# ExaScience/elprep

Measured on AMD Instinct MI355X. Metric: Mreads/s through sort+markdup+BQSR, 150bp PE, higher is better.
Workload: dtype u8/int32/int64 (integer path; float64 finalize on host)

## Files before the change

### elprep_amd/csrc/bqsr.hip

```cpp
#include <utility>

#include "bqsr_common.hpp"

namespace elp {

__global__ __launch_bounds__(256) void k_pack_reference(const uint8_t *__restrict__ ascii, int64_t len, uint8_t *__restrict__ packed, int64_t packed_bytes) {
  const int64_t i = (int64_t)blockIdx.x * blockDim.x + threadIdx.x;
  if (i >= packed_bytes) return;
  uint32_t out = 0;
  for (int h = 0; h < 2; h++) {
    const int64_t j = 2 * i + h;
    uint32_t code = 8;
    if (j < len) {
      switch (ascii[j]) {
        case 'a': case 'A': case '*': code = 0; break;
        case 'c': case 'C': code = 1; break;
        case 'g': case 'G': code = 2; break;
        case 't': case 'T': code = 3; break;
        default: code = 8;
      }
    }
    out |= code << (4 * h);
  }
  packed[i] = (uint8_t)out;
// ... 102 lines not shown
  for (int q = 6; q < ELP_NQUAL; q++)
    if ((q < 64 ? (c->qual_present[0] >> q) : (c->qual_present[1] >> (q - 64))) & 1ull) quals.push_back(q);
  if (quals.empty()) quals.push_back(6);
  return quals;
}

static int rec_buffers(elp_ctx *c, const GatherScratch &S, uint32_t *block, int mode, uint32_t ncs, RecOut *ro) {
  const uint32_t nseg = mode == 2 ? std::max<uint32_t>((uint32_t)C3_NSEG, ncs) : (uint32_t)C3_NSEG;
  BqRec *recs = nullptr;
  if (mode) ELP_TRY(scratch(c, 4, S.rec_slots(mode), &recs));
  *ro = RecOut{recs, block + S.rec_cnt, block + S.seg_base, S.other_at(mode), nseg, mode == 2 ? ncs : 0u};
  if (mode) ELP_TRY(c3_segments_launch(c, S, block, nseg, ro->ncs));
  return 0;
}

static int count_one_length(elp_ctx *c, const GatherShape &g, const GatherScratch &S, const PrologueBufs &b, const RecOut &ro, const std::vector<int> &quals,
                            unsigned long long *cycle_tbl, unsigned long long *ctx_tbl) {
  const bool split = ro.ncs != 0;
  int rsw3 = 0, rlog3 = 0;
  size_t dyn3 = 0;
  (void)count3_plan(split ? 1 : g.n_cov, (int)quals.size(), g.lmax, g.lds_count3, &rsw3, &rlog3, &dyn3, g.count3_rlog);
  QMap qm;
  memset(qm.slot, 254, sizeof qm.slot);
  for (size_t s = 0; s < quals.size(); s++) qm.slot[quals[s]] = (uint8_t)s;
  const uint4 *other = reinterpret_cast<const uint4 *>(ro.recs) + 2 * (size_t)ro.other_at;
  const uint32_t *n_other = ro.cnt + (size_t)ro.nseg * C3_CSTRIDE;
  uint32_t *cw = b.block + S.cw, *ooff = cw + CO_MAXCOV;
  ELP_HIP(c, hipMemsetAsync(cw, 0, (3 * CO_MAXCOV + 1) * sizeof(uint32_t), c->stream));
  if (split) {
    uint4 *sorted = const_cast<uint4 *>(other) + 2 * (size_t)c->n;
    ELP_TRY(c3_other_sort_launch(c, other, n_other, cw, sorted));
    other = sorted;
  }
  Count3Args A3{ro.cnt, (uint32_t)C3_CSTRIDE, ro.seg_base, reinterpret_cast<const uint4 *>(ro.recs), ro.nseg, 0, (int)ro.ncs, c->uniform_len, c->qual.p,
                c->seq4.p + elp_ctx::SEQ_FRONT, reinterpret_cast<const uint8_t *>(b.skipbits), reinterpret_cast<const uint4 *>(b.desc), c->cigar.p, b.cs_pool,
                c->d_ref_seq.p, c->d_ref_seq_len.p, g.n_cov, (int)quals.size(), g.lmax, g.max_cycle, rsw3, rlog3, cycle_tbl, ctx_tbl, c->err_flag.p};
  ELP_TRY(count3_launch(c, A3, qm, dyn3));
  A3.other = 1;
  A3.srecs = other;
  A3.seg_base = ooff;
  A3.cnt_stride = 1;
  if (split) { A3.seg_cnt = cw; A3.nseg = ro.ncs; }
  else { A3.seg_cnt = n_other; A3.nseg = 1; }
  return count3_launch(c, A3, qm, dyn3);
}

static int count_general(elp_ctx *c, const GatherShape &g, const CountPlan &p, const PrologueBufs &b, const std::vector<int> &quals,
                         unsigned long long *cycle_tbl, unsigned long long *ctx_tbl) {
  for (int cov0 = 0; cov0 < g.n_cov; cov0 += p.ncp)
    for (size_t q0 = 0; q0 < quals.size(); q0 += (size_t)p.qcap) {
      const int nqs = (int)std::min<size_t>((size_t)p.qcap, quals.size() - q0), ncov_pass = std::min(p.ncp, g.n_cov - cov0);
      QMap qm;
      memset(qm.slot, 254, sizeof qm.slot);
      for (int q : quals) qm.slot[q] = 255;
      for (int s = 0; s < nqs; s++) qm.slot[quals[q0 + s]] = (uint8_t)s;
      CountArgs A{c->n, c->qual_bytes, c->qual_off.p, c->seq_off.p, c->qual.p, c->seq4.p, b.desc, c->cigar.p, b.cs_pool,
                  reinterpret_cast<const uint8_t *>(b.skipbits), c->d_ref_seq.p, c->d_ref_seq_len.p, c->n_ref, ncov_pass, nqs, g.lmax, p.rs, g.max_cycle,
                  cycle_tbl, ctx_tbl, c->err_flag.p, c->tile_first.p, cov0};
      ELP_TRY(count_general_launch(c, A, qm, p, p.dyn(ncov_pass, nqs)));
    }
  return 0;
}

static int tables_to_host(elp_ctx *c, size_t nq, size_t nc, size_t nx, int64_t *qual_tbl, int64_t *cycle_tbl, int64_t *ctx_tbl) {
  const size_t bytes = (nq + nc + nx) * 8;
  if (bytes > c->h_pinned_cap) {
    if (c->h_pinned) (void)hipHostFree(c->h_pinned);
// ... 233 lines not shown
```

### elprep_amd/csrc/bqsr_common.hpp

```cpp
#pragma once
#include "apply_plan.hpp"
#include "bqsr_dev.hpp"
#include "bqsr_plan.hpp"
#include "flat.hpp"

namespace elp {

constexpr int MAX_DESC_READ = 65535;


constexpr int32_t BQ_NOREF = INT32_MIN;
enum : uint8_t { BQ_ELIGIBLE = 1, BQ_REVERSED = 2, BQ_LAST = 4, BQ_CIG_SCRATCH = 8, BQ_COMPLEX = 16 };
struct __attribute__((aligned(16))) BqDesc {
  int32_t D0, D1, D2;
  int32_t refid;
  uint16_t b1, b2;
  uint16_t a;
  uint16_t len;
  uint16_t left;
  uint16_t right;
  uint8_t cov;
  uint8_t fl;
  uint16_t pad;
};
// ... 192 lines not shown
  if (!general && any_ref) {
    if (P.np > 1 && !(nr & 2u)) { const int64_t d = P.v1 - vf; general |= d < -16 || d > 14; d1 = (int)d; }
    if (P.np > 2 && !(nr & 4u)) { const int64_t d = P.v2 - vf; general |= d < -16 || d > 14; d2 = (int)d; }
    if (P.np > 3 && !(nr & 8u)) { const int64_t d = P.v3 - vf; general |= d < -16 || d > 14; d3 = (int)d; }
    general |= E0 < 16 || E0 + lorig > rlen + 32;
  }
  general |= !any_ref;
  if (general) {
    fl |= RC_GENERAL;
    r.bpk = 0x3FFFFFFFu; r.dpk = 0;
  } else {
    fl |= (nr & 0xFu) << 24;
    if (P.np > 1 || (nr & 1u)) fl |= RC_MULTI;
    r.bpk = (uint32_t)(P.np > 1 ? P.s1 : 1023) | ((uint32_t)(P.np > 2 ? P.s2 : 1023) << 10) | ((uint32_t)(P.np > 3 ? P.s3 : 1023) << 20);
    r.dpk = ((uint32_t)d1 & 0xFFu) | (((uint32_t)d2 & 0xFFu) << 8) | (((uint32_t)d3 & 0xFFu) << 16);
    fl |= (E0 & 1) ? RC_PAR : 0u;
  }
  const uint64_t pq = reinterpret_cast<uint64_t>(general ? rp : rp + (E0 >> 1) - 8);
  r.ref_lo = (uint32_t)pq;
  r.ref_hi = (uint32_t)(pq >> 32);
  r.fl = fl;
  return r;
}

struct Count3Args {
  const uint32_t *seg_cnt;
  uint32_t cnt_stride;
  const uint32_t *seg_base;
  const uint4 *srecs;
  uint32_t nseg;
  int other;
  int ncs;
  uint32_t len;
  const uint8_t *qual, *seq4;
  const uint8_t *skipbits;
  const uint4 *desc;
  const uint32_t *cigar, *cig_scratch;
  uint8_t *const *ref_seq;
  const int64_t *ref_seq_len;
  int n_cov, n_q, lmax, max_cycle;
  int rsw, rlog;
  unsigned long long *cycle_tbl, *ctx_tbl;
  uint32_t *err;
};
int count3_launch(elp_ctx *c, const Count3Args &A, const QMap &qm, size_t dyn);

struct CountArgs {
  uint64_t n, qual_bytes;
  const uint64_t *qual_off, *seq_off;
  const uint8_t *qual, *seq4;
  const BqDesc *desc;
  const uint32_t *cigar, *cig_scratch;
  const uint8_t *skipbits;
  uint8_t *const *ref_seq;
  const int64_t *ref_seq_len;
  int n_ref, n_cov, n_q, lmax, rs, max_cycle;
  unsigned long long *cycle_tbl, *ctx_tbl;
  uint32_t *err;
  const uint32_t *tile_first;
  int cov0;
};

int count_general_launch(elp_ctx *c, const CountArgs &A, const QMap &qm, const CountPlan &p, size_t dyn);
int qual_from_cycle_launch(elp_ctx *c, int ncyc_g, const unsigned long long *cycle_tbl, unsigned long long *qual_tbl);
int c3_segments_launch(elp_ctx *c, const GatherScratch &S, uint32_t *block, uint32_t nseg, uint32_t ncs);
int c3_other_sort_launch(elp_ctx *c, const uint4 *other, const uint32_t *n_other, uint32_t *cw, uint4 *sorted);
// ... 30 lines not shown
```

### elprep_amd/csrc/bqsr_plan.hpp

```cpp
#pragma once
#include <algorithm>
#include <cstddef>
#include <cstdint>

namespace elp {

constexpr size_t LDS_CU = 160 * 1024;

constexpr int CT_CYC = 32, CT_XROWS = 3, CT_PAD = 64;
constexpr int C3_XROWS = 3, C3_PAD = 64;
constexpr int C3_NSEG = 64;
constexpr int C3_MAXSEG = 256;
constexpr int C3_CSTRIDE = 64;
constexpr int PF_TILES = 16;
constexpr int CO_MAXCOV = 256;

inline int count3_plan(int n_cov, int n_q, int lmax, size_t static_lds, int *rsw_out, int *rlog_out, size_t *dyn_out, int force_rlog = -1) {
  const int ncw = ((17 * 2 * lmax) >> 4) + 2;
  const size_t rows = (size_t)n_cov * (size_t)(n_q + C3_XROWS);
  for (int rlog = 5; rlog >= 1; rlog--) {
    if (force_rlog >= 0 && force_rlog != rlog) continue;
    const int rsw = ((16 << rlog) + 16 + ncw + 31) & ~31;
    const size_t dyn = (rows * (size_t)rsw + C3_PAD) * 4;
    if (dyn + static_lds <= LDS_CU && rows * (size_t)rsw * 4 < (1u << 22)) {
      *rsw_out = rsw; *rlog_out = rlog; *dyn_out = dyn;
      return 0;
    }
  }
  return 1;
}

struct GatherShape {
  int n_cov, lmax, max_cycle;
  uint32_t uniform_len;
  int count_kernel, count3_rlog;
  size_t lds_count3, lds_count, lds_count1024;
};

inline int c3_mode(const GatherShape &g, int nq) {
  if (g.count_kernel == 1 || g.uniform_len == 0 || g.lmax > g.max_cycle || g.lmax > 1022) return 0;
  int rsw = 0, rlog = 0;
  size_t dyn = 0;
  const bool all_fits = count3_plan(g.n_cov, nq, g.lmax, g.lds_count3, &rsw, &rlog, &dyn, g.count3_rlog) == 0;
  if (all_fits && (rlog >= 3 || g.n_cov == 1) && g.count_kernel != 3) return 1;
  if (g.n_cov > 1 && g.count_kernel != 2 && count3_plan(1, nq, g.lmax, g.lds_count3, &rsw, &rlog, &dyn, g.count3_rlog) == 0) return 2;
  return all_fits ? 1 : 0;
}

struct CountPlan {
  bool fits;
  int wg_per_cu;
  bool big, mg;
  int rs;
  int ncp, qcap;
  long passes;
  size_t dyn(int ncov_pass, int nqs) const { return ((size_t)ncov_pass * (size_t)(nqs + CT_XROWS) * (size_t)rs + CT_PAD) * 4; }
};
inline int count_row_words(int lmax, bool mg) {
  const int cyc = (17 * 2 * lmax) >> 4;
  return (CT_CYC + (mg ? cyc >> 1 : cyc) + 1 + 1) & ~1;
}
inline CountPlan count_general_plan(const GatherShape &g, int nq) {
// ... 57 lines not shown
```

### elprep_amd/csrc/common.hpp

```cpp
#pragma once

#include <hip/hip_runtime.h>

#include <sched.h>

#include <cstdarg>
#include <cstdint>
#include <cstdio>
#include <cstring>
#include <map>
#include <mutex>
#include <string>
#include <vector>

#include "../../include/elprep_hip.h"
#include "../../include/elprep_hip_debug.h"
#include "apply_plan.hpp"
#include "derived.hpp"

namespace elp {

constexpr int WAVE = 64;

enum : uint16_t {
// ... 175 lines not shown
  uint64_t *presort_ks = nullptr;
  int presort_idx_bits = 0;

  elp::DVec<uint16_t> snap_flag;
  elp::DVec<uint8_t> snap_qual;
  uint64_t snap_n = 0, snap_qual_bytes = 0;

  struct Tuning {
    int count_kernel = 0;
    int apply_kernel = 0;
    int count3_rlog = -1;
    int qual_hint = 0;
    int qual_hint_drop = -1;
    int pair_table_slots = 1 << 20;
    long long bgzf_piece = 1ll << 30;
    int bgzf_weak_guess = 0;
    int score_kernel = 0;
    int mate_path = 0;
    int radix_tile = 0;
    int sort_pairs = 0;
    int tie_rounds = 0;
    int exchange_piece = 0;
    int emit_pass = 0;
    int sam_pass = 0;
    long long bgzf_inflate_piece = 2ll << 30;
    int bgzf_copy_chunk = 0;
    int bgzf_tok_lds = 0;
    int bgzf_first_chunk_div = 4;
    int bgzf_fixed = 0;
    int bgzf_tok_fail_above = 0;
    int bgzf_stored = 0;
    int apply_wgs = 0;
    int count3_grid = 0;
    int presort_tile = 0;
    int side_priority = 0;
  } tune;

  elp::DVec<uint8_t> scratch[8];

  bool profiling = false;
  const char *prof_prefix = nullptr;
  std::vector<std::string> prof_names;
  std::map<std::string, int> prof_index;
  std::vector<uint64_t> prof_launches;
  std::vector<double> prof_ms;
  std::vector<elp::ProfPending> prof_pending;
};

namespace elp {

class LaneViews {
  struct Item { void *vec; void (*take_back)(void *); };
  std::vector<Item> items;

 public:
  template <class... Col>
  LaneViews(elp_ctx *shadow, elp_ctx *ctx, Col... cols) { (view(shadow->*cols, ctx->*cols), ...); }
  LaneViews(const LaneViews &) = delete;
  LaneViews &operator=(const LaneViews &) = delete;
  ~LaneViews() {
    for (const Item &it : items) it.take_back(it.vec);
  }
  template <class T>
  void view(DVec<T> &to, const DVec<T> &from, bool with_cap = false) {
    to.p = from.p;
    to.cap = with_cap ? from.cap : 0;
// ... 212 lines not shown
```

### elprep_amd/csrc/count3.hip

```cpp
#include <algorithm>

#include "bqsr_common.hpp"
#include "gload.hpp"

namespace elp {

constexpr uint32_t N1 = 0x11111111u, C3 = 0x33333333u;
constexpr int C3_NT = 1024;

template <int BYTE>
__device__ __forceinline__ uint32_t byte_shl2(uint32_t w, uint32_t two) {
  uint32_t r;
  if (BYTE == 0) asm("v_lshlrev_b32_sdwa %0, %1, %2 dst_sel:DWORD dst_unused:UNUSED_PAD src0_sel:DWORD src1_sel:BYTE_0" : "=v"(r) : "v"(two), "v"(w));
  else if (BYTE == 1) asm("v_lshlrev_b32_sdwa %0, %1, %2 dst_sel:DWORD dst_unused:UNUSED_PAD src0_sel:DWORD src1_sel:BYTE_1" : "=v"(r) : "v"(two), "v"(w));
  else if (BYTE == 2) asm("v_lshlrev_b32_sdwa %0, %1, %2 dst_sel:DWORD dst_unused:UNUSED_PAD src0_sel:DWORD src1_sel:BYTE_2" : "=v"(r) : "v"(two), "v"(w));
  else asm("v_lshlrev_b32_sdwa %0, %1, %2 dst_sel:DWORD dst_unused:UNUSED_PAD src0_sel:DWORD src1_sel:BYTE_3" : "=v"(r) : "v"(two), "v"(w));
  return r;
}
__device__ __forceinline__ uint32_t lds_read_u32(uint32_t at) { return *reinterpret_cast<const lds_u32_t *>((uintptr_t)at); }

struct BlkRec { uint32_t win, ctxw, t0, fl, bpk, dpk; };
struct BlkData {
  u32x4 q;
  uint32_t skipw;
  u32x4 s;
  u32x4 w03;
  u32x2 w45;
};

__device__ __noinline__ uint64_t c3_ref_general(const uint4 *__restrict__ desc, const uint32_t *__restrict__ cigar, const uint32_t *__restrict__ cig_scratch,
                                               uint8_t *const *__restrict__ ref_seq, const int64_t *__restrict__ ref_seq_len, uint32_t r, uint64_t S, int blo, int bhi,
                                               int cbase) {
  const uint4 dx = desc[2 * (size_t)r], dy = desc[2 * (size_t)r + 1];
  const uint32_t dfl = (dy.w >> 8) & 0xFFu;
  const int32_t refid = (int32_t)dx.w;
  const uint8_t *__restrict__ rp = ref_seq[refid];
  const int64_t rlen = ref_seq_len[refid];
  const int32_t D0 = (int32_t)dx.x, D1 = (int32_t)dx.y, D2 = (int32_t)dx.z;
  const int b1 = (int)(dy.x & 0xFFFFu), b2 = (int)(dy.x >> 16);
  uint64_t R = 0;
  if (!(dfl & BQ_COMPLEX)) {
    const int B1 = b1 - cbase, B2 = b2 - cbase;
    {
      const int hi = bhi < B1 ? bhi : B1;
      if (blo < hi) R |= (D0 == BQ_NOREF ? S : ref_nibbles(rp, rlen, (int64_t)D0 + cbase)) & nib_fill(nib_range(blo, hi));
    }
    if (B1 < bhi) {
      const int lo = blo > B1 ? blo : B1, hi = bhi < B2 ? bhi : B2;
      if (lo < hi) R |= (D1 == BQ_NOREF ? S : ref_nibbles(rp, rlen, (int64_t)D1 + cbase)) & nib_fill(nib_range(lo, hi));
      if (B2 < bhi) {
        const int lo2 = blo > B2 ? blo : B2;
        if (lo2 < bhi) R |= (D2 == BQ_NOREF ? S : ref_nibbles(rp, rlen, (int64_t)D2 + cbase)) & nib_fill(nib_range(lo2, bhi));
      }
    }
  } else {
    const uint32_t *cg = ((dfl & BQ_CIG_SCRATCH) ? cig_scratch : cigar) + (uint32_t)D0;
    R = ref_nibbles_complex(cg, b1, (int64_t)D2, cbase, blo, bhi, rp, rlen, S);
  }
  return R;
}


template <int RLOG, bool OTHER>
struct Count3 {
  const uint8_t *__restrict__ qual;
  const uint8_t *__restrict__ seq_m1;
  const uint8_t *__restrict__ skipbits;
  const uint4 *__restrict__ desc;
  const uint32_t *__restrict__ cigar;
  const uint32_t *__restrict__ cig_scratch;
  uint8_t *const *__restrict__ ref_seq;
  const int64_t *__restrict__ ref_seq_len;
  unsigned long long *cycle_tbl, *ctx_tbl;
  uint32_t k0, nb;
  int n_cov, n_q, lmax, max_cycle, rsw;
  uint32_t qrow_at, spread_at;
  const uint8_t *slot_q;
  uint32_t *tbl;
  uint32_t rpc_bytes;
  int cov_fixed;
  int t_origin;
  uint32_t rep4, two;
  uint32_t err;

  __device__ __forceinline__ bool load_data(const u32x4 &ra, const u32x4 &rb, bool on, uint32_t len, uint32_t sbytes, BlkData &d, BlkRec &f, uint32_t &qlow,
                                            uint32_t &idx) const {
    const uint32_t a = ra.z & 0xFFFFu, e = ra.z >> 16;
    f.win = ra.z; f.ctxw = ra.w; f.t0 = rb.x; f.fl = rb.y; f.bpk = rb.z; f.dpk = rb.w;
    idx = rec_idx(ra.y, rb.y, rb.w);
    const uint64_t bit = (uint64_t)idx * len + k0;
    qlow = (uint32_t)bit & 7u;
    if (!on || k0 + nb <= a || k0 >= e) return false;
    gload_x4(d.q, (uint64_t)qual + bit);
    d.skipw = 0u;
    if (OTHER && (rb.y & RC_SKIPCOL)) gload_x1(d.skipw, (uint64_t)skipbits + (bit >> 3));
    gload_x4(d.s, (uint64_t)seq_m1 + (uint64_t)idx * sbytes + (k0 >> 1));
    const uint64_t rp = ((uint64_t)ra.x | ((uint64_t)(ra.y & 0xFFFFu) << 32)) + ((rb.y & RC_GENERAL) ? 0u : (k0 >> 1));
    gload_x4(d.w03, rp);
    gload_x2(d.w45, rp + 16);
    return true;
  }

  __device__ __forceinline__ static uint64_t win_extract(const BlkData &d, int n0) {
    uint32_t x0 = d.w03.x, x1 = d.w03.y, x2 = d.w03.z, x3 = d.w03.w, x4 = d.w45.x, x5 = d.w45.y;
    asm("" : "+v"(x0), "+v"(x1), "+v"(x2), "+v"(x3), "+v"(x4), "+v"(x5));
    const bool s16 = n0 & 16, s8 = n0 & 8;
    const uint32_t y0 = s16 ? x2 : x0, y1 = s16 ? x3 : x1, y2 = s16 ? x4 : x2, y3 = s16 ? x5 : x3;
    const uint32_t z0 = s8 ? y1 : y0, z1 = s8 ? y2 : y1, z2 = s8 ? y3 : y2;
    const uint32_t sh = 4u * (uint32_t)(n0 & 7);
    return (uint64_t)__builtin_amdgcn_alignbit(z1, z0, sh) | ((uint64_t)__builtin_amdgcn_alignbit(z2, z1, sh) << 32);
  }
  __device__ __forceinline__ static uint64_t ref_pieces(const BlkData &d, uint32_t fl, uint32_t bpk, uint32_t dpk, uint64_t S, int blo, int bhi, int cbase) {
    const int par = (fl & RC_PAR) ? 1 : 0;
    const uint32_t nr = fl >> 24;
    const int f = !(nr & 1u) ? 0 : (!(nr & 2u) ? 1 : (!(nr & 4u) ? 2 : 3));
    uint64_t R = 0;
#pragma unroll
    for (int j = 0; j < 4; j++) {
      const int bj = j == 0 ? 0 : (int)((bpk >> (10 * (j - 1))) & 1023u), bn = j == 3 ? 1023 : (int)((bpk >> (10 * j)) & 1023u);
      if (j > 0 && bj == 1023) break;
      int lo = bj - cbase, hi = bn == 1023 ? bhi : bn - cbase;
      lo = lo > blo ? lo : blo;
      hi = hi < bhi ? hi : bhi;
      if (lo < hi) {
        const int dj = j == 0 ? 0 : (int)(int8_t)((dpk >> (8 * (j - 1))) & 0xFFu);
        const uint64_t piece = ((nr >> j) & 1u) ? S : win_extract(d, 16 + par + (j == f ? 0 : dj));
        R |= piece & nib_fill(nib_range(lo, hi));
      }
    }
    return R;
  }
  template <int I>
  __device__ __forceinline__ uint32_t row_of(uint32_t qw) const { return lds_read_u32(qrow_at + byte_shl2<(I & 3)>(qw, two)); }
  template <int I>
  __device__ __forceinline__ void base(uint32_t ro, uint32_t Fh, uint32_t FVh, uint32_t CXh, uint32_t t, uint32_t lrepC) {
    constexpr int sh = 4 * (I & 7);
    lds_add_u32(lshl_add_u32<2>(t >> 4, ro), bfe_u32<sh, 1>(Fh));
    lds_add_u32(ro + lshl_add_u32<RLOG + 2>(bfe_u32<sh, 4>(CXh), lrepC), bfe_u32<sh, 1>(FVh));
  }
  __device__ __forceinline__ void mismatches(uint32_t Eh, uint32_t FVh, uint32_t CXh, uint32_t qa, uint32_t qb, uint32_t tb, int st, uint32_t rowb) {
    constexpr uint32_t cxm = (uint32_t)(16 << RLOG) * 4u;
    while (Eh) {
      const uint32_t b4 = (uint32_t)__builtin_ctz(Eh);
      const uint32_t b = b4 >> 2;
      Eh &= Eh - 1u;
      const uint32_t q = (((b & 4u) ? qb : qa) >> (8u * (b & 3u))) & 0xFFu;
      if (q < 6u) continue;
      const uint32_t ro = lds_read_u32(qrow_at + 4u * q);
      const uint32_t t = tb + (uint32_t)(st * (int)b);
      lds_add_u32(ro + ((t >> 4) << 2), 0x10000u);
      if ((FVh >> b4) & 1u) lds_add_u32(ro + rowb + cxm + (((CXh >> b4) & 15u) << 2), 1u);
    }
  }

  __device__ __forceinline__ void process(const BlkRec &f, uint32_t r, const BlkData &d, uint32_t qlow) {
    const int a = (int)(f.win & 0xFFFFu), e = (int)(f.win >> 16);
    int blo = a - (int)k0, bhi = e - (int)k0;
    blo = blo > 0 ? blo : 0;
    bhi = bhi < (int)nb ? bhi : (int)nb;
    const uint32_t fl = f.fl;
    const bool rev = fl & RC_REV;
    const uint32_t ns = rev ? 12u : 4u;
    const uint32_t S_lo = __builtin_amdgcn_alignbit(d.s.y, d.s.x, 8), S_hi = __builtin_amdgcn_alignbit(d.s.z, d.s.y, 8);
    const uint32_t N_lo = __builtin_amdgcn_alignbit(d.s.y, d.s.x, ns), N_hi = __builtin_amdgcn_alignbit(d.s.z, d.s.y, ns);
    const uint32_t oS_lo = (S_lo >> 3) & N1, oS_hi = (S_hi >> 3) & N1;
    const uint32_t oN_lo = (N_lo >> 3) & N1, oN_hi = (N_hi >> 3) & N1;
    uint32_t R_lo = 0, R_hi = 0, k_lo = 0, k_hi = 0;
    const bool one_run = !OTHER || !(fl & (RC_MULTI | RC_GENERAL));
    const bool skipcol = OTHER && (fl & RC_SKIPCOL);
    if (one_run) {
      const uint32_t sh = (fl & RC_PAR) ? 4u : 0u;
      R_lo = __builtin_amdgcn_alignbit(d.w03.w, d.w03.z, sh);
      R_hi = __builtin_amdgcn_alignbit(d.w45.x, d.w03.w, sh);
      if (!skipcol) {
        k_lo = (R_lo >> 2) & N1;
        k_hi = (R_hi >> 2) & N1;
      }
    }
    if (skipcol) {
      const uint32_t sk = d.skipw >> qlow;
      k_lo |= lds_read_u32(spread_at + ((sk & 0xFFu) << 2));
      k_hi |= lds_read_u32(spread_at + ((sk >> 6) & 0x3FCu));
    }
    const uint64_t inw = nib_range(blo, bhi);
    const uint32_t F_lo = (uint32_t)inw & ~(oS_lo | k_lo), F_hi = (uint32_t)(inw >> 32) & ~(oS_hi | k_hi);
    if ((F_lo | F_hi) == 0u) return;
    if (!one_run) {
      const uint64_t S = (uint64_t)S_lo | ((uint64_t)S_hi << 32);
      const uint64_t R = (fl & RC_GENERAL) ? c3_ref_general(desc, cigar, cig_scratch, ref_seq, ref_seq_len, r, S, blo, bhi, (int)k0 - a) : ref_pieces(d, fl, f.bpk, f.dpk, S, blo, bhi, (int)k0 - a);
      R_lo = (uint32_t)R;
      R_hi = (uint32_t)(R >> 32);
    }
    const uint32_t x_lo = S_lo ^ R_lo, x_hi = S_hi ^ R_hi;
    const uint32_t E_lo = (x_lo | (x_lo >> 1) | (x_lo >> 3)) & F_lo & N1, E_hi = (x_hi | (x_hi >> 1) | (x_hi >> 3)) & F_hi & N1;
    const uint64_t cw = nib_range_clamped((int)(f.ctxw & 0xFFFFu) - (int)k0, (int)(f.ctxw >> 16) - (int)k0);
    const uint32_t FV_lo = F_lo & (uint32_t)cw & ~oN_lo, FV_hi = F_hi & (uint32_t)(cw >> 32) & ~oN_hi;
    const uint32_t rm = rev ? 0xFFFFFFFFu : 0u;
    const uint32_t CX_lo = ((N_lo & C3) | ((S_lo & C3) << 2)) ^ rm, CX_hi = ((N_hi & C3) | ((S_hi & C3) << 2)) ^ rm;
    const int st = (fl & RC_NEG) ? -17 : 17;
    const uint32_t rowb = cov_fixed >= 0 ? 0u : __umul24(fl & 0xFFu, rpc_bytes);
    const uint32_t tb = (uint32_t)((int)f.t0 + t_origin + st * (int)k0) + 4u * rowb;
    const uint32_t lrepC = rowb + rep4;
    const uint32_t ust = (uint32_t)st;
#define ELP_B3(I, RO, FH, FVH, CXH) base<I>(RO, FH, FVH, CXH, tb + (uint32_t)(I) * ust, lrepC)
    {
      const uint32_t r0 = row_of<0>(d.q.x), r1 = row_of<1>(d.q.x), r2 = row_of<2>(d.q.x), r3 = row_of<3>(d.q.x);
      const uint32_t r4 = row_of<4>(d.q.y), r5 = row_of<5>(d.q.y), r6 = row_of<6>(d.q.y), r7 = row_of<7>(d.q.y);
      ELP_B3(0, r0, F_lo, FV_lo, CX_lo); ELP_B3(1, r1, F_lo, FV_lo, CX_lo); ELP_B3(2, r2, F_lo, FV_lo, CX_lo); ELP_B3(3, r3, F_lo, FV_lo, CX_lo);
      ELP_B3(4, r4, F_lo, FV_lo, CX_lo); ELP_B3(5, r5, F_lo, FV_lo, CX_lo); ELP_B3(6, r6, F_lo, FV_lo, CX_lo); ELP_B3(7, r7, F_lo, FV_lo, CX_lo);
      __builtin_amdgcn_sched_barrier(0);
    }
    {
      const uint32_t r0 = row_of<8>(d.q.z), r1 = row_of<9>(d.q.z), r2 = row_of<10>(d.q.z), r3 = row_of<11>(d.q.z);
      const uint32_t r4 = row_of<12>(d.q.w), r5 = row_of<13>(d.q.w), r6 = row_of<14>(d.q.w), r7 = row_of<15>(d.q.w);
      ELP_B3(8, r0, F_hi, FV_hi, CX_hi); ELP_B3(9, r1, F_hi, FV_hi, CX_hi); ELP_B3(10, r2, F_hi, FV_hi, CX_hi); ELP_B3(11, r3, F_hi, FV_hi, CX_hi);
      ELP_B3(12, r4, F_hi, FV_hi, CX_hi); ELP_B3(13, r5, F_hi, FV_hi, CX_hi); ELP_B3(14, r6, F_hi, FV_hi, CX_hi); ELP_B3(15, r7, F_hi, FV_hi, CX_hi);
      __builtin_amdgcn_sched_barrier(0);
    }
#undef ELP_B3
    {
// ... 88 lines not shown
  asm volatile("" : "+v"(B.two));
  B.err = 0;
  B.cov_fixed = A.ncs ? 0 : -1;

  const uint32_t len = A.len, bpr = (len + 15u) >> 4, sbytes = (len + 1u) >> 1, RPI = C3_NT / bpr;
  const uint32_t slot = threadIdx.x / bpr, jb = threadIdx.x - slot * bpr;
  const bool lane_on = slot < RPI;
  B.k0 = 16u * jb;
  B.nb = len - B.k0 < 16u ? len - B.k0 : 16u;
  __shared__ uint32_t s_cnt[C3_MAXSEG], s_pre[C3_MAXSEG + 1], s_wsum[4];
  static_assert(sizeof(qrow) + sizeof(spread8) + sizeof(slot_q) + sizeof(s_cnt) + sizeof(s_pre) + sizeof(s_wsum) == COUNT3_LDS_ARRAYS,
                "COUNT3_LDS_ARRAYS lists the kernel's __shared__ arrays: add a new one there too");
  {
    const uint32_t my_cnt = threadIdx.x < A.nseg ? A.seg_cnt[(size_t)threadIdx.x * A.cnt_stride] : 0u;
    const uint32_t my_trips = (my_cnt + RPI - 1u) / RPI;
    uint32_t incl = my_trips;
    for (int d = 1; d < 64; d <<= 1) {
      const uint32_t v = __shfl_up(incl, d, 64);
      if ((int)(threadIdx.x & 63u) >= d) incl += v;
    }
    if (threadIdx.x < (uint32_t)C3_MAXSEG && (threadIdx.x & 63u) == 63u) s_wsum[threadIdx.x >> 6] = incl;
    __syncthreads();
    if (threadIdx.x < (uint32_t)C3_MAXSEG) {
      uint32_t off = 0;
      for (uint32_t w = 0; w < (threadIdx.x >> 6); w++) off += s_wsum[w];
      s_cnt[threadIdx.x] = my_cnt;
      s_pre[threadIdx.x] = off + incl - my_trips;
      if (threadIdx.x == (uint32_t)C3_MAXSEG - 1u) s_pre[C3_MAXSEG] = off + incl;
    }
    __syncthreads();
  }
  const uint64_t trips_all = to_sgpr(s_pre[C3_MAXSEG]);
  const uint32_t my_lo = to_sgpr((uint32_t)(trips_all * blockIdx.x / gridDim.x)), my_hi = to_sgpr((uint32_t)(trips_all * (blockIdx.x + 1ull) / gridDim.x));
  const uint32_t flush_every = 30000u / (RPI + 1u) + 1u;
  uint64_t n = 0;
  const uint8_t *seg_recs = nullptr;
  auto first_read = [&](uint64_t it) __attribute__((always_inline)) -> uint64_t { return it * RPI; };
  const uint32_t roff = slot * 32u;
  auto rec_load = [&](uint64_t it, u32x4 &za, u32x4 &zb) __attribute__((always_inline)) {
    const uint64_t r0 = first_read(it);
    if (lane_on && r0 + slot < n) {
      const uint8_t *rt = seg_recs + r0 * 32u;
      gload_x4(za, rt, roff);
      gload_x4(zb, rt, roff + 16u);
    }
  };
  auto data_load = [&](uint64_t it, const u32x4 &za, const u32x4 &zb, BlkData &d, BlkRec &f, uint32_t &qlow, uint32_t &idx) __attribute__((always_inline)) -> bool {
    const uint64_t r0 = first_read(it);
    const bool on = lane_on && r0 + slot < n;
    return B.load_data(za, zb, on, len, sbytes, d, f, qlow, idx);
  };
  auto landed = [&](BlkData &d, const u32x4 &za, const u32x4 &zb, u32x4 &ra, u32x4 &rb) __attribute__((always_inline)) {
    gwait();
    asm volatile("" : "+v"(d.q), "+v"(d.skipw), "+v"(d.s), "+v"(d.w03), "+v"(d.w45));
    ra = amov(za);
    rb = amov(zb);
  };
  BlkData dX, dY;
  dX.q = (u32x4){0, 0, 0, 0}; dX.s = dX.q; dX.w03 = dX.q; dX.w45 = (u32x2){0, 0}; dX.skipw = 0;
  dY = dX;
  BlkRec fX, fY;
  u32x4 za = (u32x4){0, 0, 0, 0}, zb = za, na = za, nb4 = za;
  uint32_t qlX = 0, qlY = 0, iX = 0, iY = 0;
  bool onX, onY = false;
  uint32_t since = 0;
  uint32_t seg = 0;
  for (uint32_t a = 0, b = A.nseg; b - a > 1u;) {
    const uint32_t md = (a + b) >> 1;
    if (s_pre[md] <= my_lo) { a = md; seg = md; } else b = md;
  }
#pragma unroll 1
  for (; seg < A.nseg; seg++) {
    const uint32_t p0 = to_sgpr(s_pre[seg]);
    if (p0 >= my_hi) break;
    const uint32_t tr = to_sgpr(s_pre[seg + 1]) - p0, cnt_s = to_sgpr(s_cnt[seg]);
    const uint32_t t0 = my_lo > p0 ? my_lo - p0 : 0u, t1 = my_hi - p0 < tr ? my_hi - p0 : tr;
    if (t0 >= t1) continue;
    const uint64_t r_first = (uint64_t)t0 * RPI, r_end = (uint64_t)t1 * RPI < (uint64_t)cnt_s ? (uint64_t)t1 * RPI : (uint64_t)cnt_s;
    n = to_sgpr(r_end - r_first);
    seg_recs = reinterpret_cast<const uint8_t *>(to_sgpr(reinterpret_cast<uint64_t>(A.srecs) + ((uint64_t)A.seg_base[seg] + r_first) * 32u));
    const uint64_t n_trips = t1 - t0;
    B.cov_fixed = A.ncs ? (int)(seg & ((uint32_t)A.ncs - 1u)) : -1;
    rec_load(0, za, zb);
    landed(dX, za, zb, na, nb4);
    onX = data_load(0, na, nb4, dX, fX, qlX, iX);
    rec_load(1, za, zb);
    landed(dX, za, zb, na, nb4);
#pragma unroll 1
    for (uint64_t it = 0; it < n_trips; it += 2) {
      {
        onY = data_load(it + 1, na, nb4, dY, fY, qlY, iY);
        rec_load(it + 2, za, zb);
// ... 43 lines not shown
```

### elprep_amd/csrc/ctx.hip

```cpp
#include "common.hpp"

namespace elp {

namespace {
constexpr size_t GUARD = 4096;
constexpr uint8_t GUARD_BYTE = 0xC3;
std::mutex guard_mu;
std::map<void *, size_t> guard_of;
int guard_check_one(void *p, size_t payload) {
  uint8_t host[GUARD];
  if (hipDeviceSynchronize() != hipSuccess || hipMemcpy(host, static_cast<uint8_t *>(p) + payload, GUARD, hipMemcpyDeviceToHost) != hipSuccess) return 0;
  for (size_t k = 0; k < GUARD; k++)
    if (host[k] != GUARD_BYTE) {
      fprintf(stderr, "[elp] ELP_DEBUG_GUARD: byte %zu behind the end of a %zu-byte device buffer was overwritten (0x%02x)\n", k, payload, host[k]);
      return 1;
    }
  return 0;
}
}
size_t debug_guard_bytes() {
  static const size_t v = [] { const char *e = getenv("ELP_DEBUG_GUARD"); return (e && *e && *e != '0') ? GUARD : (size_t)0; }();
  return v;
}
void debug_guard_arm(void *p, size_t payload) {
// ... 568 lines not shown
  if (k == "count_kernel") c->tune.count_kernel = v;
  else if (k == "apply_kernel") c->tune.apply_kernel = v;
  else if (k == "bgzf_piece") { if (value < 1) return set_error(c, ELP_ERR_ARG, "elp_set_tuning: bgzf_piece must be positive"); c->tune.bgzf_piece = value; }
  else if (k == "bgzf_weak_guess") c->tune.bgzf_weak_guess = v;
  else if (k == "score_kernel") { c->tune.score_kernel = v; c->derived.score_tuning_changed(); }
  else if (k == "count3_rlog") c->tune.count3_rlog = v;
  else if (k == "qual_hint") { c->tune.qual_hint = v; c->derived.hint_tuning_changed(); }
  else if (k == "qual_hint_drop") { c->tune.qual_hint_drop = v; c->derived.hint_tuning_changed(); }
  else if (k == "pair_table_slots") {
    if (v == 0) { c->tune.pair_table_slots = 1 << 20; return 0; }
    if (v < 2 || v > (1 << 20) || (v & (v - 1))) return set_error(c, ELP_ERR_ARG, "elp_set_tuning: pair_table_slots must be a power of two >= 2");
    c->tune.pair_table_slots = v;
  } else if (k == "mate_path") {
    if (value != 0 && value != 2) return set_error(c, ELP_ERR_ARG, "elp_set_tuning: mate_path is 0 (the library decides) or 2 (every candidate through the table)");
    c->tune.mate_path = v;
  } else if (k == "tie_rounds") c->tune.tie_rounds = v;
  else if (k == "radix_tile") c->tune.radix_tile = v;
  else if (k == "sort_pairs") c->tune.sort_pairs = v;
  else if (k == "exchange_piece") c->tune.exchange_piece = v;
  else if (k == "emit_pass") c->tune.emit_pass = v;
  else if (k == "sam_pass") c->tune.sam_pass = v;
  else if (k == "bgzf_stored") c->tune.bgzf_stored = v;
  else if (k == "bgzf_tok_fail_above") c->tune.bgzf_tok_fail_above = v;
  else if (k == "bgzf_fixed") c->tune.bgzf_fixed = v;
  else if (k == "bgzf_first_chunk_div") c->tune.bgzf_first_chunk_div = v;
  else if (k == "bgzf_tok_lds") c->tune.bgzf_tok_lds = v;
  else if (k == "bgzf_copy_chunk") c->tune.bgzf_copy_chunk = v;
  else if (k == "bgzf_inflate_piece") { if (value < 1) return set_error(c, ELP_ERR_ARG, "elp_set_tuning: bgzf_inflate_piece must be positive"); c->tune.bgzf_inflate_piece = value; }
  else if (k == "md_fused" || k == "bgzf_inflate") {
    if (value != 0) return set_error(c, ELP_ERR_ARG, "elp_set_tuning: key '%s' is retired (only 0 is accepted)", key);
  } else if (k == "apply_wgs") c->tune.apply_wgs = v;
  else if (k == "presort_tile") c->tune.presort_tile = v;
  else if (k == "count3_grid") { if (value < 0) return set_error(c, ELP_ERR_ARG, "elp_set_tuning: count3_grid must not be negative"); c->tune.count3_grid = v; }
  else if (k == "side_priority") c->tune.side_priority = v;
  else return set_error(c, ELP_ERR_ARG, "elp_set_tuning: unknown key '%s'", key);
  return 0;
}

int elp_profile_enable(elp_ctx *c, int on) {
  if (!c) return ELP_ERR_ARG;
  if (!on) { ELP_TRY(prof_flush(c)); prof_merge_side(c); }
  c->profiling = on != 0;
  for (int lane = 0; lane < 2; lane++)
    if (c->side[lane]) c->side[lane]->profiling = c->profiling;
  return 0;
}
int elp_profile_reset(elp_ctx *c) {
  if (!c) return ELP_ERR_ARG;
  ELP_TRY(prof_flush(c));
  prof_merge_side(c);
  for (auto &v : c->prof_launches) v = 0;
  for (auto &v : c->prof_ms) v = 0.0;
  return 0;
}
int elp_profile_count(elp_ctx *c) {
  if (!c) return ELP_ERR_ARG;
  if (prof_flush(c) != 0) return ELP_ERR_HIP;
  prof_merge_side(c);
  return (int)c->prof_names.size();
}
int elp_profile_get(elp_ctx *c, int index, const char **name, uint64_t *launches, double *total_ms) {
  if (!c || index < 0 || index >= (int)c->prof_names.size()) return ELP_ERR_ARG;
  if (name) *name = c->prof_names[index].c_str();
  if (launches) *launches = c->prof_launches[index];
  if (total_ms) *total_ms = c->prof_ms[index];
  return 0;
// ... 4 lines not shown
```

### elprep_amd/csrc/gload.hpp

```cpp
#pragma once
#include <cstdint>

namespace elp {

typedef uint32_t u32x4 __attribute__((ext_vector_type(4)));
typedef uint32_t u32x2 __attribute__((ext_vector_type(2)));

__device__ __forceinline__ uint32_t to_sgpr(uint32_t x) { return (uint32_t)__builtin_amdgcn_readfirstlane((int)x); }
__device__ __forceinline__ uint64_t to_sgpr(uint64_t x) { return (uint64_t)to_sgpr((uint32_t)x) | ((uint64_t)to_sgpr((uint32_t)(x >> 32)) << 32); }
__device__ __forceinline__ void gload_x4(u32x4 &v, const void *sbase, uint32_t off) {
  asm volatile("global_load_dwordx4 %0, %1, %2" : "=v"(v) : "v"(off), "s"(sbase) : "memory");
}
__device__ __forceinline__ void gload_x2(u32x2 &v, const void *sbase, uint32_t off) {
  asm volatile("global_load_dwordx2 %0, %1, %2" : "=v"(v) : "v"(off), "s"(sbase) : "memory");
}
__device__ __forceinline__ void gload_x1(uint32_t &v, const void *sbase, uint32_t off) {
  asm volatile("global_load_dword %0, %1, %2" : "=v"(v) : "v"(off), "s"(sbase) : "memory");
}
__device__ __forceinline__ void gload_x4(u32x4 &v, uint64_t addr) { asm volatile("global_load_dwordx4 %0, %1, off" : "=v"(v) : "v"(addr) : "memory"); }
__device__ __forceinline__ void gload_x1(uint32_t &v, uint64_t addr) { asm volatile("global_load_dword %0, %1, off" : "=v"(v) : "v"(addr) : "memory"); }
__device__ __forceinline__ void gload_x2(u32x2 &v, uint64_t addr) { asm volatile("global_load_dwordx2 %0, %1, off" : "=v"(v) : "v"(addr) : "memory"); }

__device__ __forceinline__ void gstore_x4(uint64_t addr, u32x4 v) { asm volatile("global_store_dwordx4 %0, %1, off" : : "v"(addr), "v"(v) : "memory"); }

__device__ __forceinline__ void gwait() { asm volatile("s_waitcnt vmcnt(0)" ::: "memory"); }
template <int N>
__device__ __forceinline__ void gwait_but() { asm volatile("s_waitcnt vmcnt(%0)" : : "n"(N) : "memory"); }
__device__ __forceinline__ uint32_t amov(uint32_t x) {
  uint32_t r;
  asm volatile("v_mov_b32 %0, %1" : "=v"(r) : "v"(x));
  return r;
}
__device__ __forceinline__ u32x4 amov(u32x4 x) { return (u32x4){amov(x.x), amov(x.y), amov(x.z), amov(x.w)}; }
__device__ __forceinline__ u32x2 amov(u32x2 x) { return (u32x2){amov(x.x), amov(x.y)}; }

}
```

Measured before the change: 2450.

## Specialize count3 block data for non-other path and derive flush interval from read length

Templates the per-block load buffer on OTHER so the common (non-other) path loads only three dwords of sequence and three dwords of reference, instead of four plus six. Skip-column and general-ref handling are compiled out there. This cuts VGPR use and memory traffic per block. It also replaces the hardcoded flush interval with one computed from the read length and a 16-bit cell maximum, and adds an optional tuning key to lower it. This could change how often LDS counters are flushed to global memory.

New measurement: 2454, median of 2. No clear change (+0.2%).

```diff
diff --git a/elprep_amd/csrc/bqsr.hip b/elprep_amd/csrc/bqsr.hip
--- a/elprep_amd/csrc/bqsr.hip
+++ b/elprep_amd/csrc/bqsr.hip
@@ -158,7 +158,7 @@
     ELP_TRY(c3_other_sort_launch(c, other, n_other, cw, sorted));
     other = sorted;
   }
-  Count3Args A3{ro.cnt, (uint32_t)C3_CSTRIDE, ro.seg_base, reinterpret_cast<const uint4 *>(ro.recs), ro.nseg, 0, (int)ro.ncs, c->uniform_len, c->qual.p,
+  Count3Args A3{ro.cnt, (uint32_t)C3_CSTRIDE, ro.seg_base, reinterpret_cast<const uint4 *>(ro.recs), ro.nseg, 0, (int)ro.ncs, c->uniform_len, count3_flush_every(c->uniform_len, c->tune.count3_flush), c->qual.p,
                 c->seq4.p + elp_ctx::SEQ_FRONT, reinterpret_cast<const uint8_t *>(b.skipbits), reinterpret_cast<const uint4 *>(b.desc), c->cigar.p, b.cs_pool,
                 c->d_ref_seq.p, c->d_ref_seq_len.p, g.n_cov, (int)quals.size(), g.lmax, g.max_cycle, rsw3, rlog3, cycle_tbl, ctx_tbl, c->err_flag.p};
   ELP_TRY(count3_launch(c, A3, qm, dyn3));
diff --git a/elprep_amd/csrc/bqsr_common.hpp b/elprep_amd/csrc/bqsr_common.hpp
--- a/elprep_amd/csrc/bqsr_common.hpp
+++ b/elprep_amd/csrc/bqsr_common.hpp
@@ -248,6 +248,7 @@
   int other;
   int ncs;
   uint32_t len;
+  uint32_t flush_every;
   const uint8_t *qual, *seq4;
   const uint8_t *skipbits;
   const uint4 *desc;
diff --git a/elprep_amd/csrc/bqsr_plan.hpp b/elprep_amd/csrc/bqsr_plan.hpp
--- a/elprep_amd/csrc/bqsr_plan.hpp
+++ b/elprep_amd/csrc/bqsr_plan.hpp
@@ -28,6 +28,13 @@
     }
   }
   return 1;
+}
+
+constexpr uint32_t C3_CELL_MAX = 65535;
+inline uint32_t count3_rpi(uint32_t len) { return 1024u / std::max<uint32_t>((len + 15u) >> 4, 1u); }
+inline uint32_t count3_flush_every(uint32_t len, int tune = 0) {
+  const uint32_t plan = std::max<uint32_t>(C3_CELL_MAX / std::max<uint32_t>(count3_rpi(len), 1u), 1u);
+  return tune > 0 ? std::min<uint32_t>((uint32_t)tune, plan) : plan;
 }
 
 struct GatherShape {
diff --git a/elprep_amd/csrc/common.hpp b/elprep_amd/csrc/common.hpp
--- a/elprep_amd/csrc/common.hpp
+++ b/elprep_amd/csrc/common.hpp
@@ -231,6 +231,7 @@
     int bgzf_stored = 0;
     int apply_wgs = 0;
     int count3_grid = 0;
+    int count3_flush = 0;
     int presort_tile = 0;
     int side_priority = 0;
   } tune;
diff --git a/elprep_amd/csrc/count3.hip b/elprep_amd/csrc/count3.hip
--- a/elprep_amd/csrc/count3.hip
+++ b/elprep_amd/csrc/count3.hip
@@ -20,12 +20,35 @@
 __device__ __forceinline__ uint32_t lds_read_u32(uint32_t at) { return *reinterpret_cast<const lds_u32_t *>((uintptr_t)at); }
 
 struct BlkRec { uint32_t win, ctxw, t0, fl, bpk, dpk; };
+template <bool OTHER>
 struct BlkData {
   u32x4 q;
   uint32_t skipw;
   u32x4 s;
   u32x4 w03;
   u32x2 w45;
+  __device__ __forceinline__ void clear() { q = (u32x4){0, 0, 0, 0}; s = q; w03 = q; w45 = (u32x2){0, 0}; skipw = 0; }
+  __device__ __forceinline__ void landed() { asm volatile("" : "+v"(q), "+v"(skipw), "+v"(s), "+v"(w03), "+v"(w45)); }
+  __device__ __forceinline__ uint32_t s0() const { return s.x; }
+  __device__ __forceinline__ uint32_t s1() const { return s.y; }
+  __device__ __forceinline__ uint32_t s2() const { return s.z; }
+  __device__ __forceinline__ uint32_t r2() const { return w03.z; }
+  __device__ __forceinline__ uint32_t r3() const { return w03.w; }
+  __device__ __forceinline__ uint32_t r4() const { return w45.x; }
+};
+template <>
+struct BlkData<false> {
+  u32x4 q;
+  u32x3 s;
+  u32x3 w;
+  __device__ __forceinline__ void clear() { q = (u32x4){0, 0, 0, 0}; s = (u32x3){0, 0, 0}; w = s; }
+  __device__ __forceinline__ void landed() { asm volatile("" : "+v"(q), "+v"(s), "+v"(w)); }
+  __device__ __forceinline__ uint32_t s0() const { return s.x; }
+  __device__ __forceinline__ uint32_t s1() const { return s.y; }
+  __device__ __forceinline__ uint32_t s2() const { return s.z; }
+  __device__ __forceinline__ uint32_t r2() const { return w.x; }
+  __device__ __forceinline__ uint32_t r3() const { return w.y; }
+  __device__ __forceinline__ uint32_t r4() const { return w.z; }
 };
 
 __device__ __noinline__ uint64_t c3_ref_general(const uint4 *__restrict__ desc, const uint32_t *__restrict__ cigar, const uint32_t *__restrict__ cig_scratch,
@@ -83,7 +106,7 @@
   uint32_t rep4, two;
   uint32_t err;
 
-  __device__ __forceinline__ bool load_data(const u32x4 &ra, const u32x4 &rb, bool on, uint32_t len, uint32_t sbytes, BlkData &d, BlkRec &f, uint32_t &qlow,
+  __device__ __forceinline__ bool load_data(const u32x4 &ra, const u32x4 &rb, bool on, uint32_t len, uint32_t sbytes, BlkData<OTHER> &d, BlkRec &f, uint32_t &qlow,
                                             uint32_t &idx) const {
     const uint32_t a = ra.z & 0xFFFFu, e = ra.z >> 16;
     f.win = ra.z; f.ctxw = ra.w; f.t0 = rb.x; f.fl = rb.y; f.bpk = rb.z; f.dpk = rb.w;
@@ -92,16 +115,22 @@
     qlow = (uint32_t)bit & 7u;
     if (!on || k0 + nb <= a || k0 >= e) return false;
     gload_x4(d.q, (uint64_t)qual + bit);
-    d.skipw = 0u;
-    if (OTHER && (rb.y & RC_SKIPCOL)) gload_x1(d.skipw, (uint64_t)skipbits + (bit >> 3));
-    gload_x4(d.s, (uint64_t)seq_m1 + (uint64_t)idx * sbytes + (k0 >> 1));
+    const uint64_t sp = (uint64_t)seq_m1 + (uint64_t)idx * sbytes + (k0 >> 1);
     const uint64_t rp = ((uint64_t)ra.x | ((uint64_t)(ra.y & 0xFFFFu) << 32)) + ((rb.y & RC_GENERAL) ? 0u : (k0 >> 1));
-    gload_x4(d.w03, rp);
-    gload_x2(d.w45, rp + 16);
+    if constexpr (OTHER) {
+      d.skipw = 0u;
+      if (rb.y & RC_SKIPCOL) gload_x1(d.skipw, (uint64_t)skipbits + (bit >> 3));
+      gload_x4(d.s, sp);
+      gload_x4(d.w03, rp);
+      gload_x2(d.w45, rp + 16);
+    } else {
+      gload_x3(d.s, sp);
+      gload_x3(d.w, rp + 8);
+    }
     return true;
   }
 
-  __device__ __forceinline__ static uint64_t win_extract(const BlkData &d, int n0) {
+  __device__ __forceinline__ static uint64_t win_extract(const BlkData<true> &d, int n0) {
     uint32_t x0 = d.w03.x, x1 = d.w03.y, x2 = d.w03.z, x3 = d.w03.w, x4 = d.w45.x, x5 = d.w45.y;
     asm("" : "+v"(x0), "+v"(x1), "+v"(x2), "+v"(x3), "+v"(x4), "+v"(x5));
     const bool s16 = n0 & 16, s8 = n0 & 8;
@@ -110,7 +139,7 @@
     const uint32_t sh = 4u * (uint32_t)(n0 & 7);
     return (uint64_t)__builtin_amdgcn_alignbit(z1, z0, sh) | ((uint64_t)__builtin_amdgcn_alignbit(z2, z1, sh) << 32);
   }
-  __device__ __forceinline__ static uint64_t ref_pieces(const BlkData &d, uint32_t fl, uint32_t bpk, uint32_t dpk, uint64_t S, int blo, int bhi, int cbase) {
+  __device__ __forceinline__ static uint64_t ref_pieces(const BlkData<true> &d, uint32_t fl, uint32_t bpk, uint32_t dpk, uint64_t S, int blo, int bhi, int cbase) {
     const int par = (fl & RC_PAR) ? 1 : 0;
     const uint32_t nr = fl >> 24;
     const int f = !(nr & 1u) ? 0 : (!(nr & 2u) ? 1 : (!(nr & 4u) ? 2 : 3));
@@ -153,7 +182,7 @@
     }
   }
 
-  __device__ __forceinline__ void process(const BlkRec &f, uint32_t r, const BlkData &d, uint32_t qlow) {
+  __device__ __forceinline__ void process(const BlkRec &f, uint32_t r, const BlkData<OTHER> &d, uint32_t qlow) {
     const int a = (int)(f.win & 0xFFFFu), e = (int)(f.win >> 16);
     int blo = a - (int)k0, bhi = e - (int)k0;
     blo = blo > 0 ? blo : 0;
@@ -161,8 +190,8 @@
     const uint32_t fl = f.fl;
     const bool rev = fl & RC_REV;
     const uint32_t ns = rev ? 12u : 4u;
-    const uint32_t S_lo = __builtin_amdgcn_alignbit(d.s.y, d.s.x, 8), S_hi = __builtin_amdgcn_alignbit(d.s.z, d.s.y, 8);
-    const uint32_t N_lo = __builtin_amdgcn_alignbit(d.s.y, d.s.x, ns), N_hi = __builtin_amdgcn_alignbit(d.s.z, d.s.y, ns);
+    const uint32_t S_lo = __builtin_amdgcn_alignbit(d.s1(), d.s0(), 8), S_hi = __builtin_amdgcn_alignbit(d.s2(), d.s1(), 8);
+    const uint32_t N_lo = __builtin_amdgcn_alignbit(d.s1(), d.s0(), ns), N_hi = __builtin_amdgcn_alignbit(d.s2(), d.s1(), ns);
     const uint32_t oS_lo = (S_lo >> 3) & N1, oS_hi = (S_hi >> 3) & N1;
     const uint32_t oN_lo = (N_lo >> 3) & N1, oN_hi = (N_hi >> 3) & N1;
     uint32_t R_lo = 0, R_hi = 0, k_lo = 0, k_hi = 0;
@@ -170,22 +199,24 @@
     const bool skipcol = OTHER && (fl & RC_SKIPCOL);
     if (one_run) {
       const uint32_t sh = (fl & RC_PAR) ? 4u : 0u;
-      R_lo = __builtin_amdgcn_alignbit(d.w03.w, d.w03.z, sh);
-      R_hi = __builtin_amdgcn_alignbit(d.w45.x, d.w03.w, sh);
+      R_lo = __builtin_amdgcn_alignbit(d.r3(), d.r2(), sh);
+      R_hi = __builtin_amdgcn_alignbit(d.r4(), d.r3(), sh);
       if (!skipcol) {
         k_lo = (R_lo >> 2) & N1;
         k_hi = (R_hi >> 2) & N1;
       }
     }
-    if (skipcol) {
-      const uint32_t sk = d.skipw >> qlow;
-      k_lo |= lds_read_u32(spread_at + ((sk & 0xFFu) << 2));
-      k_hi |= lds_read_u32(spread_at + ((sk >> 6) & 0x3FCu));
+    if constexpr (OTHER) {
+      if (skipcol) {
+        const uint32_t sk = d.skipw >> qlow;
+        k_lo |= lds_read_u32(spread_at + ((sk & 0xFFu) << 2));
+        k_hi |= lds_read_u32(spread_at + ((sk >> 6) & 0x3FCu));
+      }
     }
     const uint64_t inw = nib_range(blo, bhi);
     const uint32_t F_lo = (uint32_t)inw & ~(oS_lo | k_lo), F_hi = (uint32_t)(inw >> 32) & ~(oS_hi | k_hi);
     if ((F_lo | F_hi) == 0u) return;
-    if (!one_run) {
+    if constexpr (OTHER) if (!one_run) {
       const uint64_t S = (uint64_t)S_lo | ((uint64_t)S_hi << 32);
       const uint64_t R = (fl & RC_GENERAL) ? c3_ref_general(desc, cigar, cig_scratch, ref_seq, ref_seq_len, r, S, blo, bhi, (int)k0 - a) : ref_pieces(d, fl, f.bpk, f.dpk, S, blo, bhi, (int)k0 - a);
       R_lo = (uint32_t)R;
@@ -340,7 +371,7 @@
   }
   const uint64_t trips_all = to_sgpr(s_pre[C3_MAXSEG]);
   const uint32_t my_lo = to_sgpr((uint32_t)(trips_all * blockIdx.x / gridDim.x)), my_hi = to_sgpr((uint32_t)(trips_all * (blockIdx.x + 1ull) / gridDim.x));
-  const uint32_t flush_every = 30000u / (RPI + 1u) + 1u;
+  const uint32_t flush_every = A.flush_every;
   uint64_t n = 0;
   const uint8_t *seg_recs = nullptr;
   auto first_read = [&](uint64_t it) __attribute__((always_inline)) -> uint64_t { return it * RPI; };
@@ -353,19 +384,19 @@
       gload_x4(zb, rt, roff + 16u);
     }
   };
-  auto data_load = [&](uint64_t it, const u32x4 &za, const u32x4 &zb, BlkData &d, BlkRec &f, uint32_t &qlow, uint32_t &idx) __attribute__((always_inline)) -> bool {
+  auto data_load = [&](uint64_t it, const u32x4 &za, const u32x4 &zb, BlkData<OTHER> &d, BlkRec &f, uint32_t &qlow, uint32_t &idx) __attribute__((always_inline)) -> bool {
     const uint64_t r0 = first_read(it);
     const bool on = lane_on && r0 + slot < n;
     return B.load_data(za, zb, on, len, sbytes, d, f, qlow, idx);
   };
-  auto landed = [&](BlkData &d, const u32x4 &za, const u32x4 &zb, u32x4 &ra, u32x4 &rb) __attribute__((always_inline)) {
+  auto landed = [&](BlkData<OTHER> &d, const u32x4 &za, const u32x4 &zb, u32x4 &ra, u32x4 &rb) __attribute__((always_inline)) {
     gwait();
-    asm volatile("" : "+v"(d.q), "+v"(d.skipw), "+v"(d.s), "+v"(d.w03), "+v"(d.w45));
+    d.landed();
     ra = amov(za);
     rb = amov(zb);
   };
-  BlkData dX, dY;
-  dX.q = (u32x4){0, 0, 0, 0}; dX.s = dX.q; dX.w03 = dX.q; dX.w45 = (u32x2){0, 0}; dX.skipw = 0;
+  BlkData<OTHER> dX, dY;
+  dX.clear();
   dY = dX;
   BlkRec fX, fY;
   u32x4 za = (u32x4){0, 0, 0, 0}, zb = za, na = za, nb4 = za;
diff --git a/elprep_amd/csrc/ctx.hip b/elprep_amd/csrc/ctx.hip
--- a/elprep_amd/csrc/ctx.hip
+++ b/elprep_amd/csrc/ctx.hip
@@ -624,6 +624,7 @@
   } else if (k == "apply_wgs") c->tune.apply_wgs = v;
   else if (k == "presort_tile") c->tune.presort_tile = v;
   else if (k == "count3_grid") { if (value < 0) return set_error(c, ELP_ERR_ARG, "elp_set_tuning: count3_grid must not be negative"); c->tune.count3_grid = v; }
+  else if (k == "count3_flush") { if (value < 0) return set_error(c, ELP_ERR_ARG, "elp_set_tuning: count3_flush must not be negative"); c->tune.count3_flush = v; }
   else if (k == "side_priority") c->tune.side_priority = v;
   else return set_error(c, ELP_ERR_ARG, "elp_set_tuning: unknown key '%s'", key);
   return 0;
diff --git a/elprep_amd/csrc/gload.hpp b/elprep_amd/csrc/gload.hpp
--- a/elprep_amd/csrc/gload.hpp
+++ b/elprep_amd/csrc/gload.hpp
@@ -4,12 +4,16 @@
 namespace elp {
 
 typedef uint32_t u32x4 __attribute__((ext_vector_type(4)));
+typedef uint32_t u32x3 __attribute__((ext_vector_type(3)));
 typedef uint32_t u32x2 __attribute__((ext_vector_type(2)));
 
 __device__ __forceinline__ uint32_t to_sgpr(uint32_t x) { return (uint32_t)__builtin_amdgcn_readfirstlane((int)x); }
 __device__ __forceinline__ uint64_t to_sgpr(uint64_t x) { return (uint64_t)to_sgpr((uint32_t)x) | ((uint64_t)to_sgpr((uint32_t)(x >> 32)) << 32); }
 __device__ __forceinline__ void gload_x4(u32x4 &v, const void *sbase, uint32_t off) {
   asm volatile("global_load_dwordx4 %0, %1, %2" : "=v"(v) : "v"(off), "s"(sbase) : "memory");
+}
+__device__ __forceinline__ void gload_x3(u32x3 &v, const void *sbase, uint32_t off) {
+  asm volatile("global_load_dwordx3 %0, %1, %2" : "=v"(v) : "v"(off), "s"(sbase) : "memory");
 }
 __device__ __forceinline__ void gload_x2(u32x2 &v, const void *sbase, uint32_t off) {
   asm volatile("global_load_dwordx2 %0, %1, %2" : "=v"(v) : "v"(off), "s"(sbase) : "memory");
@@ -18,6 +22,7 @@
   asm volatile("global_load_dword %0, %1, %2" : "=v"(v) : "v"(off), "s"(sbase) : "memory");
 }
 __device__ __forceinline__ void gload_x4(u32x4 &v, uint64_t addr) { asm volatile("global_load_dwordx4 %0, %1, off" : "=v"(v) : "v"(addr) : "memory"); }
+__device__ __forceinline__ void gload_x3(u32x3 &v, uint64_t addr) { asm volatile("global_load_dwordx3 %0, %1, off" : "=v"(v) : "v"(addr) : "memory"); }
 __device__ __forceinline__ void gload_x1(uint32_t &v, uint64_t addr) { asm volatile("global_load_dword %0, %1, off" : "=v"(v) : "v"(addr) : "memory"); }
 __device__ __forceinline__ void gload_x2(u32x2 &v, uint64_t addr) { asm volatile("global_load_dwordx2 %0, %1, off" : "=v"(v) : "v"(addr) : "memory"); }
 
```
